# HaoxiangYou/Q_Learning_with_HJB

Measured on AMD Instinct MI355X. Metric: env-steps/sec (batched HJB rollouts), cartpole batch=2^20, higher is better.
Workload: dtype f32; 1 GPU; cartpole balancing + vhjb controller (BASELINE configs[1]); batch_per_gpu=1048576, global_batch=1048576, state_dim=4, control_dim=1, integrator=euler, mlp=4-128-128-64 relu, no bias, parallelism=env-shard x1, no data-path collective

## Files before the change

### q_learning_with_hjb_amd/csrc/hjbx_mlp_host.hpp

```cpp
#pragma once
#include <type_traits>

#include "hjbx_host.hpp"
#include "hjbx_mlp_kernels.hpp"
#include "hjbx_hessian_kernels.hpp"

inline hjbx_net make_net(const hjbx_mlp* mlp) {
    return hjbx_net{0, mlp->activation, mlp->h1, mlp->h2, mlp->h3, mlp->mean, mlp->std, mlp->xf, mlp->eps_scalar, (const float*)mlp->W1,
                    (const float*)mlp->W2, (const float*)mlp->W3, nullptr, nullptr, nullptr, nullptr, nullptr};
}
inline hjbx_net make_net(const hjbx_softpd_mlp* mlp) {
    return hjbx_net{1, mlp->activation, mlp->h1, mlp->h2, mlp->h3, mlp->mean, mlp->std, mlp->xf, 0.0, (const float*)mlp->W1, (const float*)mlp->W2,
                    (const float*)mlp->W3, (const float*)mlp->b1, (const float*)mlp->b2, (const float*)mlp->b3, (const float*)mlp->w4, (const float*)mlp->b4};
}

template <int N> inline MlpP<N> make_mlp_params(const hjbx_net& net) {
    MlpP<N> p;
    for (int k = 0; k < N; ++k) { p.mean[k] = (float)net.mean[k]; p.istd[k] = (float)(1.0 / net.std[k]); p.xf[k] = (float)net.xf[k]; }
    p.eps_s = (float)net.eps_scalar;
    return p;
}

template <typename Head> inline Head make_head(const hjbx_net& net) {
    if constexpr (std::is_same<Head, MlpHeadSoft>::value) return MlpHeadSoft{net.b1, net.b2, net.b3, net.w4, net.b4};
    else return MlpHeadPd{};
}

static constexpr int kEmptyCall = 1;

inline int check_features(const char* who, const hjbx_net& net) {
    if (net.h1 != kH1 || net.h2 != kH2 || net.h3 != kH3)
        return hjbx_set_error(HJBX_EUNSUPPORTED, "%s: features must be [128,128,64], got [%d,%d,%d]", who, net.h1, net.h2, net.h3);
    if (net.activation != HJBX_ACT_RELU && net.activation != HJBX_ACT_TANH && net.activation != HJBX_ACT_SIN)
        return hjbx_set_error(HJBX_EINVAL, "%s: unknown activation %d", who, net.activation);
    return HJBX_OK;
}
inline int check_std(const char* who, const hjbx_net& net, int n) {
    for (int k = 0; k < n; ++k)
        if (!(net.std[k] != 0.0)) return hjbx_set_error(HJBX_EINVAL, "%s: normalization_std[%d] is zero", who, k);
    return HJBX_OK;
}
inline bool state_rows_aligned(const void* p, const hjbx_system* sys) { return aligned_rows(p, (size_t)sys->n * sizeof(float), 7u); }
inline int check_net(const char* who, const hjbx_system* sys, const hjbx_net& net) {
    if (net.soft) {
        if (!net.W1 || !net.b1 || !net.W2 || !net.b2 || !net.W3 || !net.b3 || !net.w4 || !net.b4)
            return hjbx_set_error(HJBX_EINVAL, "%s: NULL weight or bias pointer", who);
        if (sys->kind == HJBX_SYS_USER && !hjbx_user_matrix_cores(sys))
            return hjbx_set_error(HJBX_EUNSUPPORTED, "%s: the matrix-core kernels exist for the built-in systems only", who);
    }
    return check_features(who, net);
}

inline int check_value_grad(const char* who, const hjbx_system* sys, const hjbx_net& net, const float* x, const float* V, const float* g, int64_t B) {
    if (B < 0) return hjbx_set_error(HJBX_EINVAL, "%s: negative batch size", who);
    if (B == 0 || (!V && !g)) return kEmptyCall;
    if (net.soft ? !x : (!x || !net.W1 || !net.W2 || !net.W3))
        return hjbx_set_error(HJBX_EINVAL, net.soft ? "%s: NULL x" : "%s: NULL x or weight pointer", who);
    if (int rc = check_net(who, sys, net)) return rc;
    if (!state_rows_aligned(x, sys) || (g && !state_rows_aligned(g, sys)))
        return hjbx_set_error(HJBX_EINVAL, "%s: x / gradV must be aligned to their row vector width", who);
    return check_std(who, net, sys->n);
}

inline int check_value_hessian(const char* who, const hjbx_system* sys, const hjbx_net& net, const float* x, const float* H, const float* dy, int64_t B) {
    if (B < 0) return hjbx_set_error(HJBX_EINVAL, "%s: negative batch size", who);
    if (B == 0 || (!H && !dy)) return kEmptyCall;
    if (!x || !net.W1 || !net.W2 || !net.W3 || (net.soft && (!net.b1 || !net.b2 || !net.b3 || !net.w4 || !net.b4)))
        return hjbx_set_error(HJBX_EINVAL, net.soft ? "%s: NULL x, weight or bias pointer" : "%s: NULL x or weight pointer", who);
    if (sys->kind == HJBX_SYS_USER && !hjbx_user_matrix_cores(sys))
        return hjbx_set_error(HJBX_EUNSUPPORTED, "%s: user-defined systems are not supported unless the handle has asked for the matrix-core kernels "
                                                 "(hjbx_system_enable_matrix_cores)", who);
    if (int rc = check_features(who, net)) return rc;
    if (!state_rows_aligned(x, sys) || (reinterpret_cast<uintptr_t>(H) & 15u) || (reinterpret_cast<uintptr_t>(dy) & 15u))
        return hjbx_set_error(HJBX_EINVAL, net.soft ? "%s: x must be aligned to its row vector width, H to 16 bytes"
                                                    : "%s: x must be aligned to its row vector width, H and dy_dx to 16 bytes", who);
    return check_std(who, net, sys->n);
}

inline int check_rollout(const char* who, const hjbx_system* sys, const hjbx_task* task, const hjbx_net& net, const hjbx_rollout_args& a) {
    if (int rc = check_task(task)) return rc;
    if (a.B < 0 || a.n_steps < 0 || a.t_first < 0 || a.T_max < 0) return hjbx_set_error(HJBX_EINVAL, "%s: negative size or step index", who);
    if (int rc = check_integrator(sys, a.integrator, who)) return rc;
    if (a.B == 0) return kEmptyCall;
    if (!a.x || !a.cost || !a.done || !a.done_step || (!net.soft && (!net.W1 || !net.W2 || !net.W3)))
        return hjbx_set_error(HJBX_EINVAL, net.soft ? "%s: x, cost, done and done_step must be non-NULL" : "%s: x, cost, done, done_step and the weights must be non-NULL", who);
    if (!a.workspace || (reinterpret_cast<uintptr_t>(a.workspace) & 15u))
        return hjbx_set_error(HJBX_EINVAL, "%s: workspace must be a 16-byte aligned device buffer of hjbx_rollout_workspace_bytes() zero-filled bytes", who);
    if (int rc = check_net(who, sys, net)) return rc;
    if (!state_rows_aligned(a.x, sys) || (a.traj && !state_rows_aligned(a.traj, sys)) || (a.x_out && !state_rows_aligned(a.x_out, sys)) ||
        (a.u_log && !aligned_rows(a.u_log, (size_t)sys->m * sizeof(float))))
        return hjbx_set_error(HJBX_EINVAL, "%s: x / traj / x_out / u_log must be aligned to their row vector width", who);
    return check_std(who, net, sys->n);
}

inline int mlp_persistent_grid(int64_t B, int per_group, int64_t* ngroups, int64_t* grid, const char* who) {
    *ngroups = (B + per_group - 1) / per_group;
    const int n_cu = hjbx_device_cus();
    if (n_cu <= 0) return hjbx_set_error(HJBX_ENODEVICE, "%s: no HIP device", who);
    *grid = *ngroups < n_cu ? *ngroups : n_cu;
    return HJBX_OK;
}

inline int mlp_rollout_grid(int64_t B, int64_t* ngroups, int64_t* grid, int* sched, const char* who) {
    if (int rc = mlp_persistent_grid(B, 32, ngroups, grid, who)) return rc;
    *sched = hjbx_option_value(HJBX_OPT_ROLLOUT_SCHEDULE);
    *grid += hjbx_option_value(HJBX_OPT_ROLLOUT_EXTRA_WORKGROUPS);
    if (*grid > kMaxGrid) *grid = kMaxGrid;
    return HJBX_OK;
}

template <typename S, int TL, int WAVES, int ACT, int ARITH, typename Head>
int launch_value_grad(S sys, const hjbx_net& net, const float* x, float* V, float* g, int64_t B, void* st, const char* who) {
    const MlpP<S::N> p = make_mlp_params<S::N>(net);
    int64_t ngroups = 0, grid = 0;
    if (int rc = mlp_persistent_grid(B, 32 * TL, &ngroups, &grid, who)) return rc;
    hipLaunchKernelGGL((k_value_grad_mfma<S, TL, WAVES, ACT, ARITH, Head>), dim3((unsigned)grid), dim3(WAVES * 64), 0, (hipStream_t)st, sys, p, net.W1,
                       net.W2, net.W3, x, V, g, B, ngroups, make_head<Head>(net));
    hipError_t e = hipGetLastError();
    if (e != hipSuccess) return hjbx_set_error(HJBX_EHIP, "%s: %s", who, hipGetErrorString(e));
    return HJBX_OK;
}

template <typename S, int ACT, typename Head>
int launch_value_hessian(S sys, const hjbx_net& net, const float* x, float* H, float* dy, int64_t B, void* st, const char* who) {
    const MlpP<S::N> p = make_mlp_params<S::N>(net);
    int64_t ngroups = 0, grid = 0;
    if (int rc = mlp_persistent_grid(B, 32 / S::N, &ngroups, &grid, who)) return rc;
    hipLaunchKernelGGL((k_value_hessian<S, kHessWaves, ACT, Head>), dim3((unsigned)grid), dim3(kHessWaves * 64), 0, (hipStream_t)st, sys, p, net.W1,
                       net.W2, net.W3, x, H, dy, B, ngroups, make_head<Head>(net));
    hipError_t e = hipGetLastError();
    if (e != hipSuccess) return hjbx_set_error(HJBX_EHIP, "%s: %s", who, hipGetErrorString(e));
    return HJBX_OK;
}

template <typename S, int WAVES, int ACT, int ARITH, typename Head>
int launch_rollout(const hjbx_system* sysh, S sys, const hjbx_task* task, const hjbx_net& net, const hjbx_rollout_args& a, const char* who) {
    constexpr int N = S::N, M = S::M;
    const MlpP<N> p = make_mlp_params<N>(net);
    const auto tk = make_task<float, N, M>(task);
    const auto lim = make_limits<float, M>(sysh);
    RolloutOut<N, M> o{a.traj, a.u_log, a.cost, a.done, a.resid, a.done_step, a.x_out};
    int64_t ngroups = 0, grid = 0;
    int sched = 0;
    if (int rc = mlp_rollout_grid(a.B, &ngroups, &grid, &sched, who)) return rc;
    auto launch = [&](auto integ) {
        hipLaunchKernelGGL((k_vhjb_rollout_mfma<decltype(integ)::value, S, WAVES, ACT, ARITH, Head>), dim3((unsigned)grid), dim3(WAVES * 64), 0,
                           (hipStream_t)a.stream, sys, p, tk, lim, net.W1, net.W2, net.W3, a.t_first, a.n_steps, a.T_max, a.x, a.env_order, o, a.B, ngroups,
                           (unsigned*)a.workspace, sched, make_head<Head>(net));
    };
    if (a.integrator == HJBX_EULER) launch(std::integral_constant<int, 0>{});
    else if (a.integrator == HJBX_RK4) launch(std::integral_constant<int, 1>{});
    else if constexpr (S::kHasZoh) launch(std::integral_constant<int, 2>{});
    hipError_t e = hipGetLastError();
    if (e != hipSuccess) return hjbx_set_error(HJBX_EHIP, "%s: %s", who, hipGetErrorString(e));
    return HJBX_OK;
}

template <typename Go> int dispatch_value_system(const hjbx_system* sys, const char* who, Go go) {
    switch (sys->kind) {
    case HJBX_SYS_CARTPOLE: return go(Cartpole<float>{});
#if !defined(HJBX_MLP_DEV) || defined(HJBX_MLP_DEV_QUAD2D)
    case HJBX_SYS_QUAD2D: return go(Quad2D<float>{});
#endif
#ifndef HJBX_MLP_DEV
    case HJBX_SYS_LINEAR:
        if (sys->n == 2) return go(Linear<float, 2, 1>{});
        if (sys->n == 4) return go(Linear<float, 4, 1>{});
        if (sys->n == 6) return go(Linear<float, 6, 2>{});
        break;
    case HJBX_SYS_ACROBOT: return go(Acrobot<float>{});
    case HJBX_SYS_NEARHOVER: return go(NearHover<float>{});
#endif
    }
    return hjbx_set_error(HJBX_EUNSUPPORTED, "%s: no kernel for system kind %d with n=%d", who, sys->kind, sys->n);
}
template <int TL, int WAVES, int ACT, int ARITH, typename Head>
int dispatch_value_grad(const hjbx_system* sys, const hjbx_net& net, const float* x, float* V, float* g, int64_t B, void* st, const char* who) {
    return dispatch_value_system(sys, who, [&](auto s) { return launch_value_grad<decltype(s), TL, WAVES, ACT, ARITH, Head>(s, net, x, V, g, B, st, who); });
}
template <int ACT, typename Head>
int dispatch_value_hessian(const hjbx_system* sys, const hjbx_net& net, const float* x, float* H, float* dy, int64_t B, void* st, const char* who) {
    return dispatch_value_system(sys, who, [&](auto s) { return launch_value_hessian<decltype(s), ACT, Head>(s, net, x, H, dy, B, st, who); });
}

template <int WAVES, int ACT, int ARITH, typename Head>
int dispatch_rollout(const hjbx_system* sys, const hjbx_task* task, const hjbx_net& net, const hjbx_rollout_args& a, const char* who) {
    int rc = HJBX_EUNSUPPORTED;
    const bool ok = with_system<float>(sys, [&](auto S) {
        using SS = decltype(S);
#ifdef HJBX_MLP_DEV
        if constexpr (std::is_same<SS, Cartpole<float>>::value)
#else
        if constexpr (SS::N % 2 == 0)
#endif
            rc = launch_rollout<SS, WAVES, ACT, ARITH, Head>(sys, S, task, net, a, who);
    });
    if (!ok || rc == HJBX_EUNSUPPORTED) return hjbx_set_error(HJBX_EUNSUPPORTED, "%s: no kernel for system kind %d with n=%d m=%d", who, sys->kind, sys->n, sys->m);
    return rc;
}

using mlp_value_grad_fn = int(const hjbx_system* sys, const hjbx_net& net, const float* x, float* V, float* g, int64_t B, void* stream, const char* who);
using mlp_rollout_fn = int(const hjbx_system* sys, const hjbx_task* task, const hjbx_net& net, const hjbx_rollout_args& a, const char* who);
using mlp_value_hessian_fn = int(const hjbx_system* sys, const hjbx_net& net, const float* x, float* H, float* dy, int64_t B, void* stream, const char* who);
#define HJBX_MLP_SYM2(prefix, name, v) prefix##name##v
#define HJBX_MLP_SYM(prefix, name, v) HJBX_MLP_SYM2(prefix, name, v)
#define HJBX_MLP_DECLARE_VARIANT(prefix, v)                                                          \
    __attribute__((visibility("hidden"))) mlp_value_grad_fn HJBX_MLP_SYM(prefix, _value_grad_act, v); \
    __attribute__((visibility("hidden"))) mlp_rollout_fn HJBX_MLP_SYM(prefix, _rollout_act, v);
#define HJBX_MLP_DEFINE_VARIANT(prefix, v, TL, WAVES, ACT, ARITH, Head)                                                                            \
    int HJBX_MLP_SYM(prefix, _value_grad_act, v)(const hjbx_system* sys, const hjbx_net& net, const float* x, float* V, float* g, int64_t B,        \
                                                 void* stream, const char* who) {                                                                  \
        return dispatch_value_grad<TL, WAVES, ACT, ARITH, Head>(sys, net, x, V, g, B, stream, who);                                                \
    }                                                                                                                                              \
    int HJBX_MLP_SYM(prefix, _rollout_act, v)(const hjbx_system* sys, const hjbx_task* task, const hjbx_net& net, const hjbx_rollout_args& a,       \
                                              const char* who) {                                                                                   \
        return dispatch_rollout<WAVES, ACT, ARITH, Head>(sys, task, net, a, who);                                                                  \
    }
#define HJBX_HESS_DECLARE_VARIANT(prefix, v) __attribute__((visibility("hidden"))) mlp_value_hessian_fn HJBX_MLP_SYM(prefix, _value_hessian_act, v);
#define HJBX_HESS_DEFINE_VARIANT(prefix, v, ACT, Head)                                                                                              \
    int HJBX_MLP_SYM(prefix, _value_hessian_act, v)(const hjbx_system* sys, const hjbx_net& net, const float* x, float* H, float* dy, int64_t B,    \
                                                    void* stream, const char* who) {                                                               \
        return dispatch_value_hessian<ACT, Head>(sys, net, x, H, dy, B, stream, who);                                                              \
    }
```

### q_learning_with_hjb_amd/csrc/hjbx_mlp_kernels.hpp

```cpp
#pragma once
#include <hip/hip_runtime.h>
#include <type_traits>

#include <cstddef>

#include "hjbx_internal.hpp"
#include "hjbx_systems.hpp"
#include "hjbx_mlp_core.hpp"
#include "hjbx_mlp_x3.hpp"
#include "hjbx_mlp_h2.hpp"

using namespace hjbx;

struct MlpHeadPd {
    static constexpr bool kSoft = false;
    template <int N, int AR> using Lds = typename MlpArith<AR>::template Lds<N>;
};
struct MlpHeadSoft {
    static constexpr bool kSoft = true;
    template <int N, int AR> using Lds = MlpLdsSoft<N>;
    const float *b1, *b2, *b3, *w4, *b4;
};

template <typename S, int TL, int WAVES, int ACT, int AR, typename HEAD = MlpHeadPd>
__global__ __launch_bounds__(WAVES * 64, WAVES / 4) void k_value_grad_mfma(S sys, MlpP<S::N> p, const float* __restrict__ W1g,
                                                                         const float* __restrict__ W2g, const float* __restrict__ W3g,
                                                                         const float* __restrict__ x, float* __restrict__ Vout,
                                                                         float* __restrict__ gout, int64_t B, int64_t ngroups, HEAD head) {
    constexpr int N = S::N;
    static_assert(N % 2 == 0, "state dimension must be even (k-steps of 2)");
    static_assert(AR == 0 || TL == 1, "the split-operand chains hold one tile per wave");
    __shared__ __attribute__((aligned(256))) typename HEAD::template Lds<N, AR> L;
    const int tid = threadIdx.x;
    if (tid == 0) L.next = WAVES;
#ifdef HJBX_DIAG_CLOCK
    const unsigned long long tentry = __builtin_amdgcn_s_memrealtime();
#endif
    MlpArith<AR>::template fill<N, WAVES * 64>(L, W1g, W2g, W3g, tid);
    if constexpr (HEAD::kSoft) mlp_fill_bias<WAVES * 64>(L.bias, head.b1, head.b2, head.b3, head.w4, head.b4, tid);
    __syncthreads();
    const int lane = tid & 63, wave = tid >> 6;
    const auto c = [&] { return MlpArith<AR>::template ctx<N>(L, lane); }();
    const int i = c.i, h = c.h;

    const int64_t groups_per_wg = (ngroups + gridDim.x - 1) / gridDim.x;
    const int64_t g_begin = (int64_t)blockIdx.x * groups_per_wg;
    const int64_t g_end = (g_begin + groups_per_wg < ngroups) ? g_begin + groups_per_wg : ngroups;

    auto load_rows = [&](int64_t grp, float (&dst)[TL][N]) {
#pragma unroll
        for (int t = 0; t < TL; ++t) {
            const int64_t en = (grp * TL + t) * 32 + i;
            load_sample<N>(x, p, en, grp < g_end && en < B, dst[t]);
        }
    };

    int64_t grp = g_begin + wave;
#ifdef HJBX_DIAG_CLOCK
    const unsigned long long t0c = __builtin_amdgcn_s_memtime(), t0r = __builtin_amdgcn_s_memrealtime();
#endif
    float xs[TL][N], xn[TL][N];
    load_rows(grp, xs);
    for (; grp < g_end;) {
        asm volatile("" ::: "memory");
        int nxt = 0;
        if (lane == 0) nxt = atomicAdd(&L.next, 1);
        const int64_t grp_next = g_begin + __builtin_amdgcn_readfirstlane(nxt);
        load_rows(grp_next, xn);

        float V[TL], g[TL][N];
        if constexpr (HEAD::kSoft) mlp_value_grad<S, TL, ACT, true>(sys, p, c, xs, gout != nullptr, V, g, &L.bias);
        else MlpArith<AR>::template value_grad<S, TL, ACT>(sys, p, c, xs, gout != nullptr, V, g);
#pragma unroll
        for (int t = 0; t < TL; ++t) {
            const int64_t env = (grp * TL + t) * 32 + i;
            if (env < B && h == 0) {
#ifndef HJBX_DIAG_CLOCK
                if (Vout) Vout[env] = V[t];
#endif
                if (gout) store_row<N>(gout, env, g[t]);
            }
#pragma unroll
            for (int k = 0; k < N; ++k) xs[t][k] = xn[t][k];
        }
        grp = grp_next;
    }
#ifdef HJBX_DIAG_CLOCK
    {
        const unsigned long long t1c = __builtin_amdgcn_s_memtime(), t1r = __builtin_amdgcn_s_memrealtime();
        if (Vout && gout && lane == 0) {
            float* d = Vout + 4 * ((int64_t)blockIdx.x * WAVES + wave);
            d[0] = (float)(t1c - t0c); d[1] = (float)(t1r - t0r);
            d[2] = (float)(t0r - tentry); d[3] = (float)(tentry & 0xFFFFFFull);
        }
    }
#endif
}

template <int N, int M> struct RolloutOut {
    float* traj;
    float* u_log;
    float* cost;
    float* done;
    float* resid;
    int32_t* done_step;
    float* x_out;
};

static constexpr int kWsQueue = 0;
static constexpr int kWsStarted = 32;
static constexpr int kWsExited = 64;
static constexpr int kWsFlags = 96;
static constexpr int kMaxGrid = 1024;
static constexpr int kWsOpen = kWsFlags + kMaxGrid;
static constexpr int kWsWords = kWsOpen + kMaxGrid;
#define HJBX_RLX_AGENT __ATOMIC_RELAXED, __HIP_MEMORY_SCOPE_AGENT

template <int INTEG, typename S, int WAVES, int ACT, int AR, typename HEAD = MlpHeadPd>
__global__ __launch_bounds__(WAVES * 64, WAVES / 4) void k_vhjb_rollout_mfma(S sys_k, MlpP<S::N> p_k, TaskP<float, S::N, S::M> tk_k,
                                                                           Limits<float, S::M> lim_k, const float* __restrict__ W1g,
                                                                           const float* __restrict__ W2g, const float* __restrict__ W3g,
                                                                           int t_first, int n_steps, int T_max, const float* x ,
                                                                           const int32_t* __restrict__ order, RolloutOut<S::N, S::M> o, int64_t B,
                                                                           int64_t ngroups, unsigned* ws, int sched, HEAD head) {
    constexpr int N = S::N, M = S::M;
    static_assert(N % 2 == 0, "state dimension must be even (k-steps of 2)");
    __shared__ __attribute__((aligned(256))) typename HEAD::template Lds<N, AR> L;
    __shared__ __attribute__((aligned(16))) unsigned char sys_raw[sizeof(S)];
    S& sys_s = *reinterpret_cast<S*>(sys_raw);
    __shared__ MlpP<N> p_s;
    __shared__ TaskP<float, N, M> tk_s;
    __shared__ Limits<float, M> lim_s;
    const int tid = threadIdx.x;
    __shared__ int q_next[4];
    __shared__ int waves_done;
    __shared__ unsigned my_flag;
    if (tid < 4) q_next[tid] = WAVES / 4;
    if (tid == 0) {
        waves_done = 0;
        unsigned seen = 0u;
        __hip_atomic_compare_exchange_strong(ws + kWsFlags + blockIdx.x, &seen, 1u, __ATOMIC_RELAXED, HJBX_RLX_AGENT);
        my_flag = seen;
        __hip_atomic_fetch_add(ws + kWsStarted, 1u, HJBX_RLX_AGENT);
        sys_s = sys_k; p_s = p_k; tk_s = tk_k; lim_s = lim_k;
    }
    MlpArith<AR>::template fill<N, WAVES * 64>(L, W1g, W2g, W3g, tid);
    if constexpr (HEAD::kSoft) mlp_fill_bias<WAVES * 64>(L.bias, head.b1, head.b2, head.b3, head.w4, head.b4, tid);
    __syncthreads();
    const S& sys = sys_s;
    const MlpP<N>& p = p_s;
    const TaskP<float, N, M>& tk = tk_s;
    const Limits<float, M>& lim = lim_s;
    const int lane = tid & 63, wave = __builtin_amdgcn_readfirstlane(tid >> 6);
    const unsigned my_flag_u = (unsigned)__builtin_amdgcn_readfirstlane((int)my_flag);
    const auto c = [&] { return MlpArith<AR>::template ctx<N>(L, lane); }();
    const int i = c.i, h = c.h;
    const int simd = wave & 3;
    const int G = (int)gridDim.x;
    const int64_t picks_per_wg = (ngroups + G - 1) / G;
    auto group_of = [&](int w, int64_t pick) -> int64_t {
        if (pick >= picks_per_wg) return -1;
        const int64_t g = order ? (int64_t)w + pick * G : (int64_t)w * picks_per_wg + pick;
        return g < ngroups ? g : -1;
    };
    int victim = -1;
    auto next_group = [&]() -> int64_t {
        if (sched == 1) {
            unsigned t = 0;
            if (lane == 0) t = __hip_atomic_fetch_add(ws + kWsQueue, 1u, HJBX_RLX_AGENT);
            const int64_t g = (int64_t)G * WAVES + (unsigned)__builtin_amdgcn_readfirstlane((int)t);
            return g < ngroups ? g : -1;
        }
        if (victim < 0) {
            int nxt = 0;
            if (lane == 0) nxt = atomicAdd(&q_next[simd], 1);
            const int64_t g = my_flag_u == 0u ? group_of(blockIdx.x, simd + 4 * (int64_t)__builtin_amdgcn_readfirstlane(nxt)) : -1;
            if (g >= 0) return g;
            victim = 0;
            unsigned started = 0;
            if (lane == 0) started = __hip_atomic_load(ws + kWsStarted, HJBX_RLX_AGENT);
            if (__builtin_amdgcn_readfirstlane((int)started) >= G) victim = G;
        }
        while (victim < G) {
            const int w = victim + lane;
            unsigned f = 1u;
            if (w < G) {
                f = __hip_atomic_load(ws + kWsFlags + w, HJBX_RLX_AGENT);
                if (f == 0u && __hip_atomic_compare_exchange_strong(ws + kWsFlags + w, &f, 2u, __ATOMIC_RELAXED, HJBX_RLX_AGENT)) f = 2u;
            }
            unsigned long long open = __builtin_amdgcn_ballot_w64(f == 2u);
            while (open) {
                const int b = __builtin_ctzll(open);
                unsigned t = 0;
                if (lane == 0) t = __hip_atomic_fetch_add(ws + kWsOpen + victim + b, 1u, HJBX_RLX_AGENT);
                const int64_t g = group_of(victim + b, (int64_t)(unsigned)__builtin_amdgcn_readfirstlane((int)t));
                if (g >= 0) { victim += b; return g; }
                open &= open - 1;
            }
            victim = (victim + 64 < G) ? victim + 64 : G;
        }
        return -1;
    };
    int64_t grp;
    if (sched == 1) grp = (int64_t)blockIdx.x * WAVES + wave < ngroups ? (int64_t)blockIdx.x * WAVES + wave : -1;
    else grp = my_flag_u == 0u ? group_of(blockIdx.x, wave) : -1;
    if (grp < 0) grp = next_group();
    while (grp >= 0) {
        const int64_t slot = grp * 32 + i;
        const bool valid = slot < B;
        int64_t env = valid ? (order ? (int64_t)order[slot] : slot) : 0;
        env = env < 0 ? 0 : (env >= B ? B - 1 : env);
        const bool writer = valid && h == 0;
        float xs[1][N];
        int32_t ds = 0;
        if (valid) {
            load_row<N>(x, env, xs[0]);
            ds = o.done_step[env];
        } else {
#pragma unroll
            for (int k = 0; k < N; ++k) xs[0][k] = p.xf[k];
        }
        if (o.traj && writer) store_row<N>(o.traj, env, xs[0]);
        for (int k = 0; k < n_steps; ++k) {
            asm volatile("" ::: "memory");
            float xo[N], u[M], cst, dn, res;
            if (__builtin_amdgcn_ballot_w64(ds < 0) == 0) {
#pragma unroll
                for (int q = 0; q < N; ++q) xo[q] = xs[0][q];
#pragma unroll
                for (int j = 0; j < M; ++j) u[j] = 0.0f;
                cst = dn = res = 0.0f;
            } else {
                float V[1], g[1][N];
                if constexpr (HEAD::kSoft) mlp_value_grad<S, 1, ACT, true>(sys, p, c, xs, true, V, g, &L.bias);
                else MlpArith<AR>::template value_grad<S, 1, ACT>(sys, p, c, xs, true, V, g);
                vhjb_step_env<INTEG>(sys, tk, lim, t_first + k, T_max, o.resid != nullptr, xs[0], g[0], ds, xo, u, cst, dn, res);
            }
            if (writer) {
                const int64_t row = (int64_t)k * B + env;
                o.cost[row] = cst;
                o.done[row] = dn;
                if (o.resid) o.resid[row] = res;
                if (o.u_log) store_row<M>(o.u_log + (int64_t)k * B * M, env, u);
                if (o.traj) store_row<N>(o.traj + (int64_t)(k + 1) * B * N, env, xo);
            }
#pragma unroll
            for (int q = 0; q < N; ++q) xs[0][q] = xo[q];
        }
        if (writer) {
            o.done_step[env] = ds;
            if (o.x_out) store_row<N>(o.x_out, env, xs[0]);
        }
        grp = next_group();
    }
    int lastw = 0;
    if (lane == 0 && atomicAdd(&waves_done, 1) == WAVES - 1) lastw = __hip_atomic_fetch_add(ws + kWsExited, 1u, HJBX_RLX_AGENT) == (unsigned)(G - 1);
    if (__builtin_amdgcn_readfirstlane(lastw)) {
        for (int w = lane; w < kWsWords; w += 64)
            if (w < kWsFlags || (w - kWsFlags) % kMaxGrid < G) __hip_atomic_store(ws + w, 0u, HJBX_RLX_AGENT);
    }
}
```

### q_learning_with_hjb_amd/csrc/hjbx_user.hip

```cpp
#include <hip/hip_runtime.h>
#include <hip/hiprtc.h>

#include <dlfcn.h>
#include <elf.h>

#include <cstdio>
#include <cstring>
#include <map>
#include <mutex>
#include <new>
#include <string>
#include <vector>

#include "hjbx_internal.hpp"
#include "hjbx_host.hpp"
#include "hjbx_mlp_kernels.hpp"
#include "hjbx_mlp_host.hpp"

#define HJBX_EMBEDDED_HEADERS(X)                                                    \
    X(hjbx_src_systems, "hjbx_systems.hpp", "hjbx_systems.hpp")                     \
    X(hjbx_src_stream, "hjbx_stream_kernels.hpp", "hjbx_stream_kernels.hpp")        \
    X(hjbx_src_user, "hjbx_user_kernels.hpp", "hjbx_user_kernels.hpp")              \
    X(hjbx_src_user_mlp, "hjbx_user_mlp_kernels.hpp", "hjbx_user_mlp_kernels.hpp")  \
    X(hjbx_src_mlp_core, "hjbx_mlp_core.hpp", "hjbx_mlp_core.hpp")                  \
    X(hjbx_src_mlp_kernels, "hjbx_mlp_kernels.hpp", "hjbx_mlp_kernels.hpp")         \
    X(hjbx_src_mlp_x3, "hjbx_mlp_x3.hpp", "hjbx_mlp_x3.hpp")                        \
    X(hjbx_src_mlp_h2, "hjbx_mlp_h2.hpp", "hjbx_mlp_h2.hpp")                        \
    X(hjbx_src_train_coop, "hjbx_train_coop_kernels.hpp", "hjbx_train_coop_kernels.hpp") \
    X(hjbx_src_user_train, "hjbx_user_train_kernels.hpp", "hjbx_user_train_kernels.hpp") \
    X(hjbx_src_hessian_kernels, "hjbx_hessian_kernels.hpp", "hjbx_hessian_kernels.hpp") \
    X(hjbx_src_user_hessian, "hjbx_user_hessian_kernels.hpp", "hjbx_user_hessian_kernels.hpp") \
    X(hjbx_src_abi, "../../include/hjbx.h", "hjbx.h")
#if !defined(__HIP_DEVICE_COMPILE__)
#ifndef HJBX_CSRC_DIR
#error "compile hjbx_user.hip with -DHJBX_CSRC_DIR=\"<absolute path of csrc>\""
#endif
#define HJBX_EMBED(sym, file, name)                                                                                               \
    asm(".pushsection .rodata\n.global " #sym "\n.type " #sym ", @object\n" #sym ":\n.incbin \"" HJBX_CSRC_DIR "/" file "\"\n.byte 0\n" \
        ".popsection\n");
HJBX_EMBEDDED_HEADERS(HJBX_EMBED)
#undef HJBX_EMBED
#endif
#define HJBX_DECLARE(sym, file, name) extern "C" const char sym[];
HJBX_EMBEDDED_HEADERS(HJBX_DECLARE)
#undef HJBX_DECLARE

static const char kStubRuntime[] = "// hip/hip_runtime.h: provided by hiprtc itself\n";
static const char kStubStdint[] =
    "#pragma once\n"
    "typedef signed char int8_t; typedef unsigned char uint8_t; typedef short int16_t; typedef unsigned short uint16_t;\n"
    "typedef int int32_t; typedef unsigned int uint32_t; typedef long int64_t; typedef unsigned long uint64_t; typedef unsigned long uintptr_t;\n";
static const char kStubStddef[] =
    "#pragma once\n"
    "typedef unsigned long size_t;\n"
    "#ifndef offsetof\n#define offsetof(t, m) __builtin_offsetof(t, m)\n#endif\n";
static const char kStubTypeTraits[] =
    "#pragma once\n"
    "namespace std {\n"
    "template <bool C, class A, class B> struct conditional { using type = A; };\n"
    "template <class A, class B> struct conditional<false, A, B> { using type = B; };\n"
    "template <bool C, class A, class B> using conditional_t = typename conditional<C, A, B>::type;\n"
    "template <class T, T v> struct integral_constant { static constexpr T value = v; };\n"
    "}\n";
static const char kStubInternal[] = "#pragma once\n#include \"hjbx.h\"\n";

namespace {
struct Rtc {
    decltype(&hiprtcCreateProgram) create = nullptr;
    decltype(&hiprtcCompileProgram) compile = nullptr;
    decltype(&hiprtcGetProgramLogSize) log_size = nullptr;
    decltype(&hiprtcGetProgramLog) log = nullptr;
    decltype(&hiprtcGetCodeSize) code_size = nullptr;
    decltype(&hiprtcGetCode) code = nullptr;
    decltype(&hiprtcDestroyProgram) destroy = nullptr;
    decltype(&hiprtcAddNameExpression) add_name = nullptr;
    decltype(&hiprtcGetLoweredName) lowered = nullptr;
    bool ok = false;
};

const Rtc& rtc() {
    static Rtc r;
    static std::once_flag once;
    std::call_once(once, [] {
        void* h = nullptr;
        for (const char* name : {"libhiprtc.so.7", "libhiprtc.so", "/opt/rocm/lib/libhiprtc.so"}) {
            h = dlopen(name, RTLD_NOW | RTLD_GLOBAL);
            if (h) break;
        }
        if (!h) return;
#define HJBX_SYM(field, sym) r.field = reinterpret_cast<decltype(r.field)>(dlsym(h, #sym))
        HJBX_SYM(create, hiprtcCreateProgram); HJBX_SYM(compile, hiprtcCompileProgram); HJBX_SYM(log_size, hiprtcGetProgramLogSize);
        HJBX_SYM(log, hiprtcGetProgramLog); HJBX_SYM(code_size, hiprtcGetCodeSize); HJBX_SYM(code, hiprtcGetCode);
        HJBX_SYM(destroy, hiprtcDestroyProgram); HJBX_SYM(add_name, hiprtcAddNameExpression); HJBX_SYM(lowered, hiprtcGetLoweredName);
#undef HJBX_SYM
        r.ok = r.create && r.compile && r.log_size && r.log && r.code_size && r.code && r.destroy && r.add_name && r.lowered;
    });
    return r;
}

thread_local std::string g_compile_log;

struct UserUnit {
    std::vector<char> code;
    hipModule_t mod[kMaxDevices] = {};
    std::map<std::string, hipFunction_t> fn[kMaxDevices];
    int state = 0, status = HJBX_OK;
    std::string error, log;
    std::string kernel[4];
};

struct UserProgram {
    std::mutex mu;
    UserUnit stream;
    std::string source;
    int user_kind = 0, n = 0, m = 0, np = 1;
    std::mutex mc_mu;
    bool matrix_cores = false;
    UserUnit mc[2][3];
    std::mutex train_mu;
    UserUnit train[3];
    std::mutex hess_mu;
    UserUnit hess[2][3];
};

int compile_unit(const Rtc& R, const char* who, const char* top, const char* unit_name, const std::string& snippet, int user_kind, int n, int m,
                 int np, const std::vector<std::string>& extra, const std::vector<const char*>& name_exprs, UserUnit* out) {
#define HJBX_TEXT(sym, file, name) sym,
#define HJBX_NAME(sym, file, name) name,
    const char* headers[] = {HJBX_EMBEDDED_HEADERS(HJBX_TEXT) kStubInternal, snippet.c_str(), kStubRuntime, kStubStdint, kStubStddef, kStubStddef,
                             kStubTypeTraits};
    const char* names[] = {HJBX_EMBEDDED_HEADERS(HJBX_NAME) "hjbx_internal.hpp", "hjbx_user_snippet.hpp", "hip/hip_runtime.h", "stdint.h", "stddef.h",
                           "cstddef", "type_traits"};
#undef HJBX_TEXT
#undef HJBX_NAME
    static_assert(sizeof(headers) == sizeof(names), "one name per header");
    hiprtcProgram prog = nullptr;
    if (R.create(&prog, top, unit_name, (int)(sizeof(headers) / sizeof(headers[0])), headers, names) != HIPRTC_SUCCESS)
        return hjbx_set_error(HJBX_EHIP, "%s: hiprtcCreateProgram failed", who);
    for (const char* e : name_exprs)
        if (R.add_name(prog, e) != HIPRTC_SUCCESS) { R.destroy(&prog); return hjbx_set_error(HJBX_EHIP, "%s: hiprtcAddNameExpression(%s) failed", who, e); }
    std::vector<std::string> o = {"--offload-arch=gfx950", "-O3", "-std=c++17", "-ffp-contract=on", "-DHJBX_USER_N=" + std::to_string(n),
                                  "-DHJBX_USER_M=" + std::to_string(m), "-DHJBX_USER_NP=" + std::to_string(np),
                                  "-DHJBX_USER_KIND=" + std::to_string(user_kind)};
    o.insert(o.end(), extra.begin(), extra.end());
    std::vector<const char*> opts;
    for (const std::string& f : o) opts.push_back(f.c_str());
    const hiprtcResult rc = R.compile(prog, (int)opts.size(), opts.data());
    size_t ls = 0;
    if (R.log_size(prog, &ls) == HIPRTC_SUCCESS && ls > 1) {
        g_compile_log.resize(ls);
        if (R.log(prog, &g_compile_log[0]) != HIPRTC_SUCCESS) g_compile_log.clear();
    }
    if (rc != HIPRTC_SUCCESS) {
        R.destroy(&prog);
        return hjbx_set_error(HJBX_EINVAL, "%s: the device source does not compile (hjbx_last_compile_log has the compiler's messages): %.300s", who,
                              g_compile_log.c_str());
    }
    size_t cs = 0;
    if (R.code_size(prog, &cs) != HIPRTC_SUCCESS || cs == 0) { R.destroy(&prog); return hjbx_set_error(HJBX_EHIP, "%s: no code object", who); }
    out->code.resize(cs);
    hiprtcResult rg = R.code(prog, out->code.data());
    for (size_t i = 0; rg == HIPRTC_SUCCESS && i < name_exprs.size() && i < 4; ++i) {
        const char* low = nullptr;
        rg = R.lowered(prog, name_exprs[i], &low);
        if (rg == HIPRTC_SUCCESS && low) out->kernel[i] = low;
    }
    R.destroy(&prog);
    if (rg != HIPRTC_SUCCESS) { out->code.clear(); return hjbx_set_error(HJBX_EHIP, "%s: hiprtcGetCode / hiprtcGetLoweredName failed", who); }
    return HJBX_OK;
}

long kernel_scratch_bytes(const std::vector<char>& code, const std::string& kernel) {
    Elf64_Ehdr eh;
    if (code.size() < sizeof eh) return -1;
    memcpy(&eh, code.data(), sizeof eh);
    if (memcmp(eh.e_ident, ELFMAG, SELFMAG) != 0 || eh.e_ident[EI_CLASS] != ELFCLASS64 || eh.e_shentsize != sizeof(Elf64_Shdr)) return -1;
    if (eh.e_shoff > code.size() || (size_t)eh.e_shnum * sizeof(Elf64_Shdr) > code.size() - eh.e_shoff) return -1;
    std::vector<Elf64_Shdr> sh(eh.e_shnum);
    if (eh.e_shnum) memcpy(sh.data(), code.data() + eh.e_shoff, sh.size() * sizeof(Elf64_Shdr));
    auto inside = [&](const Elf64_Shdr& s) { return s.sh_offset <= code.size() && s.sh_size <= code.size() - s.sh_offset; };
    const std::string want = kernel + ".kd";
    for (const Elf64_Shdr& st : sh) {
        if ((st.sh_type != SHT_SYMTAB && st.sh_type != SHT_DYNSYM) || st.sh_link >= sh.size() || !inside(st) || !inside(sh[st.sh_link])) continue;
        const Elf64_Shdr& str = sh[st.sh_link];
        for (size_t k = 0; k + sizeof(Elf64_Sym) <= st.sh_size; k += sizeof(Elf64_Sym)) {
            Elf64_Sym sym;
            memcpy(&sym, code.data() + st.sh_offset + k, sizeof sym);
            if (sym.st_name >= str.sh_size || sym.st_shndx >= sh.size()) continue;
            const char* nm = code.data() + str.sh_offset + sym.st_name;
            if (strnlen(nm, str.sh_size - sym.st_name) != want.size() || memcmp(nm, want.data(), want.size()) != 0) continue;
            const Elf64_Shdr& sec = sh[sym.st_shndx];
            if (!inside(sec) || sym.st_value < sec.sh_addr || sym.st_value - sec.sh_addr + 8 > sec.sh_size) return -1;
            uint32_t priv = 0;
            memcpy(&priv, code.data() + sec.sh_offset + (sym.st_value - sec.sh_addr) + 4, 4);
            return (long)priv;
        }
    }
    return -1;
}

int launch_unit(UserProgram* u, UserUnit& unit, const char* kernel, unsigned grid, unsigned block, void** args, void* stream, const char* who) {
    const int dev = hjbx_current_device();
    if (dev < 0) return hjbx_set_error(HJBX_ENODEVICE, "%s: no HIP device", who);
    hipFunction_t f = nullptr;
    {
        std::lock_guard<std::mutex> lock(u->mu);
        if (!unit.mod[dev]) {
            const hipError_t e = hipModuleLoadData(&unit.mod[dev], unit.code.data());
            if (e != hipSuccess) { unit.mod[dev] = nullptr; return hjbx_set_error(HJBX_EHIP, "hipModuleLoadData: %s", hipGetErrorString(e)); }
        }
        auto it = unit.fn[dev].find(kernel);
        if (it == unit.fn[dev].end()) {
            const hipError_t e = hipModuleGetFunction(&f, unit.mod[dev], kernel);
            if (e != hipSuccess) return hjbx_set_error(HJBX_EHIP, "hipModuleGetFunction(%s): %s", kernel, hipGetErrorString(e));
            unit.fn[dev][kernel] = f;
        } else {
            f = it->second;
        }
    }
    const hipError_t e = hipModuleLaunchKernel(f, grid, 1, 1, block, 1, 1, 0, (hipStream_t)stream, args, nullptr);
    if (e != hipSuccess) return hjbx_set_error(HJBX_EHIP, "%s: %s", who, hipGetErrorString(e));
    return HJBX_OK;
}

void unload_unit(UserUnit& unit) {
    for (int d = 0; d < kMaxDevices; ++d)
        if (unit.mod[d]) (void)hipModuleUnload(unit.mod[d]);
}

struct UnitSpec {
    const char *top, *name;
    std::vector<std::string> flags;
    std::vector<const char*> kernels, labels;
    std::string variant;
    const char* budget;
};

template <typename MakeSpec> int lazy_unit(UserProgram* u, UserUnit& unit, MakeSpec&& make_spec, const char* who, UserUnit** out) {
    if (unit.state == 0) {
        const UnitSpec spec = make_spec();
        g_compile_log.clear();
        const Rtc& R = rtc();
        int rc = compile_unit(R, who, spec.top, spec.name, u->source, u->user_kind, u->n, u->m, u->np, spec.flags, spec.kernels, &unit);
        for (size_t k = 0; rc == HJBX_OK && k < spec.kernels.size(); ++k) {
            const long scratch = kernel_scratch_bytes(unit.code, unit.kernel[k]);
            if (scratch < 0) rc = hjbx_set_error(HJBX_EHIP, "%s: kernel %s is missing from the compiled code object", who, unit.kernel[k].c_str());
            else if (scratch > 0)
                rc = hjbx_set_error(HJBX_EUNSUPPORTED, "%s: the %s kernel of this user system (n=%d m=%d, %s) needs %ld bytes of scratch: its code does not fit %s",
                                    who, spec.labels[k], u->n, u->m, spec.variant.c_str(), scratch, spec.budget);
        }
        unit.state = rc == HJBX_OK ? 1 : -1;
        unit.status = rc;
        unit.log = g_compile_log;
        if (rc != HJBX_OK) {
            char msg[512];
            hjbx_last_error(msg, sizeof msg);
            unit.error = msg;
            unit.code.clear();
        }
    }
    if (unit.state < 0) {
        g_compile_log = unit.log;
        return hjbx_set_error(unit.status, "%s", unit.error.c_str());
    }
    *out = &unit;
    return HJBX_OK;
}

int matrix_core_unit(const hjbx_system* s, int soft, int act, const char* who, UserUnit** out) {
    UserProgram* u = s->kind == HJBX_SYS_USER ? static_cast<UserProgram*>(s->user) : nullptr;
    if (!u) return hjbx_set_error(HJBX_EINVAL, "%s: not a user-defined system", who);
    if (soft < 0 || soft > 1 || act < 0 || act > 2) return hjbx_set_error(HJBX_EINVAL, "%s: unknown head %d / activation %d", who, soft, act);
    std::lock_guard<std::mutex> lock(u->mc_mu);
    if (!u->matrix_cores)
        return hjbx_set_error(HJBX_EUNSUPPORTED, "%s: this user-defined system has not asked for the matrix-core kernels (hjbx_system_enable_matrix_cores)", who);
    return lazy_unit(u, u->mc[soft][act], [&] { return
                     UnitSpec{"#include \"hjbx_user_mlp_kernels.hpp\"\n", "hjbx_user_matrix_cores.hip",
                              {"-DHJBX_USER_MLP_ACT=" + std::to_string(act), "-DHJBX_USER_MLP_SOFT=" + std::to_string(soft)},
                              {"HJBX_UM_VALUE_GRAD", "HJBX_UM_ROLLOUT_EULER", "HJBX_UM_ROLLOUT_RK4"}, {"value-gradient", "Euler rollout", "RK4 rollout"},
                              "activation " + std::to_string(act) + (soft ? ", soft-PD head" : ", PD head"), "the 256 registers of the matrix-core kernels"}; },
                     who, out);
}

int train_unit(const hjbx_system* s, int act, const char* who, UserUnit** out) {
    UserProgram* u = s->kind == HJBX_SYS_USER ? static_cast<UserProgram*>(s->user) : nullptr;
    if (!u) return hjbx_set_error(HJBX_EINVAL, "%s: not a user-defined system", who);
    if (act < 0 || act > 2) return hjbx_set_error(HJBX_EINVAL, "%s: unknown activation %d", who, act);
    if (s->n % 2)
        return hjbx_set_error(HJBX_EUNSUPPORTED, "%s: the fused parameter gradient needs an even state dimension (k-steps of 2), got n=%d", who, s->n);
    if (!hjbx_user_matrix_cores(s))
        return hjbx_set_error(HJBX_EUNSUPPORTED, "%s: this user-defined system has not asked for the matrix-core kernels (hjbx_system_enable_matrix_cores)", who);
    if (act == HJBX_ACT_SIN && s->n > 4)
        return hjbx_set_error(HJBX_EUNSUPPORTED, "%s: the sin network's fused parameter gradient exists for n <= 4 (n = %d)", who, s->n);
    std::lock_guard<std::mutex> lock(u->train_mu);
    return lazy_unit(u, u->train[act], [&] { return
                     UnitSpec{"#include \"hjbx_user_train_kernels.hpp\"\n", "hjbx_user_train.hip", {"-DHJBX_USER_MLP_ACT=" + std::to_string(act)},
                              {"HJBX_UT_M0_PS1", "HJBX_UT_M0_PS4", "HJBX_UT_M1_PS1", "HJBX_UT_M1_PS4"},
                              {"k_train_coop<mode 0, PS 1>", "k_train_coop<mode 0, PS 4>", "k_train_coop<mode 1, PS 1>", "k_train_coop<mode 1, PS 4>"},
                              "activation " + std::to_string(act),
                              "the 512 registers of the cooperative parameter-gradient kernel; the fused parameter gradient is refused for this system"}; },
                     who, out);
}

int hessian_unit(const hjbx_system* s, int soft, int act, const char* who, UserUnit** out) {
    UserProgram* u = s->kind == HJBX_SYS_USER ? static_cast<UserProgram*>(s->user) : nullptr;
    if (!u) return hjbx_set_error(HJBX_EINVAL, "%s: not a user-defined system", who);
    if (soft < 0 || soft > 1 || act < 0 || act > 2) return hjbx_set_error(HJBX_EINVAL, "%s: unknown head %d / activation %d", who, soft, act);
    if (!hjbx_user_matrix_cores(s))
        return hjbx_set_error(HJBX_EUNSUPPORTED, "%s: this user-defined system has not asked for the matrix-core kernels (hjbx_system_enable_matrix_cores)", who);
    if (soft && act == HJBX_ACT_RELU)
        return hjbx_set_error(HJBX_EUNSUPPORTED, "%s: the Hessian of a soft-PD ReLU network is identically zero (H is filled with zeros): there is no kernel and no code object", who);
    std::lock_guard<std::mutex> lock(u->hess_mu);
    return lazy_unit(u, u->hess[soft][act], [&] { return
                     UnitSpec{"#include \"hjbx_user_hessian_kernels.hpp\"\n", "hjbx_user_hessian.hip",
                              {"-DHJBX_USER_MLP_ACT=" + std::to_string(act), "-DHJBX_USER_MLP_SOFT=" + std::to_string(soft)},
                              {"HJBX_UH_VALUE_HESSIAN"}, {"value-Hessian"},
                              "activation " + std::to_string(act) + (soft ? ", soft-PD head" : ", PD head"), "the 512 registers of the Hessian kernel"}; },
                     who, out);
}
}

extern "C" size_t hjbx_last_compile_log(char* buf, size_t buflen) {
    const size_t len = g_compile_log.size();
    if (buf && buflen) {
        const size_t n = len < buflen - 1 ? len : buflen - 1;
        memcpy(buf, g_compile_log.data(), n);
        buf[n] = '\0';
    }
    return len;
}

void hjbx_user_release(void* up) {
    UserProgram* u = static_cast<UserProgram*>(up);
    if (!u) return;
    unload_unit(u->stream);
    for (auto& head : u->mc)
        for (UserUnit& unit : head) unload_unit(unit);
    for (UserUnit& unit : u->train) unload_unit(unit);
    for (auto& head : u->hess)
        for (UserUnit& unit : head) unload_unit(unit);
    delete u;
}

extern "C" int hjbx_system_create_from_source(int user_kind, const char* device_source, int n, int m, double dt, const double* umin,
                                              const double* umax, const double* params, int n_params, hjbx_system** out) {
    if (!out) return hjbx_set_error(HJBX_EINVAL, "out is NULL");
    *out = nullptr;
    g_compile_log.clear();
    if (user_kind != HJBX_USER_AFFINE && user_kind != HJBX_USER_MANIPULATOR) return hjbx_set_error(HJBX_EINVAL, "unknown user system kind %d", user_kind);
    if (!device_source || !umin || !umax) return hjbx_set_error(HJBX_EINVAL, "device_source / umin / umax must be non-NULL");
    if (n < 1 || n > HJBX_MAX_N || m < 1 || m > HJBX_MAX_M) return hjbx_set_error(HJBX_EINVAL, "user system needs 1<=n<=%d, 1<=m<=%d", HJBX_MAX_N, HJBX_MAX_M);
    if (user_kind == HJBX_USER_MANIPULATOR && n % 2) return hjbx_set_error(HJBX_EINVAL, "a manipulator state is (q, dq): n must be even, got %d", n);
    if (n_params < 0 || n_params > HJBX_USER_MAX_PARAMS || (n_params > 0 && !params))
        return hjbx_set_error(HJBX_EINVAL, "user system takes 0..%d parameters", HJBX_USER_MAX_PARAMS);
    if (!(dt > 0) || !(dt < 1e300)) return hjbx_set_error(HJBX_EINVAL, "dt must be positive and finite");
    for (int j = 0; j < m; ++j)
        if (!(umin[j] <= umax[j])) return hjbx_set_error(HJBX_EINVAL, "umin[%d] > umax[%d]", j, j);
    const Rtc& R = rtc();
    if (!R.ok) {
        const char* why = dlerror();
        return hjbx_set_error(HJBX_EUNSUPPORTED, "hjbx_system_create_from_source: libhiprtc.so could not be loaded (%s)", why ? why : "symbols missing");
    }
    UserProgram* u = new (std::nothrow) UserProgram();
    if (!u) return hjbx_set_error(HJBX_EINVAL, "out of host memory");
    u->source = device_source; u->user_kind = user_kind; u->n = n; u->m = m; u->np = n_params > 0 ? n_params : 1;
    if (int rc = compile_unit(R, "hjbx_system_create_from_source", "#include \"hjbx_user_kernels.hpp\"\n", "hjbx_user_system.hip", u->source, user_kind,
                              n, m, u->np, {}, {}, &u->stream)) {
        delete u;
        return rc;
    }
    hjbx_system* s = new_system(HJBX_SYS_USER, n, m, dt, umin, umax, params, n_params, u);
    if (!s) { delete u; return hjbx_set_error(HJBX_EINVAL, "out of host memory"); }
    *out = s;
    return HJBX_OK;
}

extern "C" int hjbx_system_enable_matrix_cores(hjbx_system* sys) {
    if (!sys) return hjbx_set_error(HJBX_EINVAL, "hjbx_system_enable_matrix_cores: system handle is NULL");
    UserProgram* u = sys->kind == HJBX_SYS_USER ? static_cast<UserProgram*>(sys->user) : nullptr;
    if (!u) return hjbx_set_error(HJBX_EINVAL, "hjbx_system_enable_matrix_cores: a built-in system has its matrix-core kernels already (user-defined systems only)");
    if (sys->n % 2)
        return hjbx_set_error(HJBX_EUNSUPPORTED, "hjbx_system_enable_matrix_cores: the matrix-core kernels need an even state dimension (k-steps of 2), got n=%d", sys->n);
    if (sys->n > HJBX_MAX_N || sys->m > HJBX_MAX_M)
        return hjbx_set_error(HJBX_EUNSUPPORTED, "hjbx_system_enable_matrix_cores: the matrix-core kernels take n<=%d, m<=%d", HJBX_MAX_N, HJBX_MAX_M);
    std::lock_guard<std::mutex> lock(u->mc_mu);
    u->matrix_cores = true;
    return HJBX_OK;
}

bool hjbx_user_matrix_cores(const hjbx_system* s) {
    UserProgram* u = s && s->kind == HJBX_SYS_USER ? static_cast<UserProgram*>(s->user) : nullptr;
    if (!u) return false;
    std::lock_guard<std::mutex> lock(u->mc_mu);
    return u->matrix_cores;
}

extern "C" int hjbx_system_matrix_cores(const hjbx_system* sys) { return hjbx_user_matrix_cores(sys) ? 1 : 0; }

extern "C" size_t hjbx_system_code_object(const hjbx_system* sys, int which, void* buf, size_t len) {
    UserProgram* u = sys && sys->kind == HJBX_SYS_USER ? static_cast<UserProgram*>(sys->user) : nullptr;
    if (!u) { hjbx_set_error(HJBX_EINVAL, "hjbx_system_code_object: not a user-defined system"); return 0; }
    const UserUnit* unit = &u->stream;
    if (which != HJBX_CODE_STREAMING) {
        if (which < 1 || which > 15) { hjbx_set_error(HJBX_EINVAL, "hjbx_system_code_object: unknown code object %d", which); return 0; }
        UserUnit* mc = nullptr;
        if (which >= 10) {
            if (hessian_unit(sys, (which - 10) / 3, (which - 10) % 3, "hjbx_system_code_object", &mc) != HJBX_OK) return 0;
        } else if (which >= 7) {
            if (train_unit(sys, which - 7, "hjbx_system_code_object", &mc) != HJBX_OK) return 0;
        } else if (matrix_core_unit(sys, (which - 1) / 3, (which - 1) % 3, "hjbx_system_code_object", &mc) != HJBX_OK) {
            return 0;
        }
        unit = mc;
    }
    if (buf && len) memcpy(buf, unit->code.data(), len < unit->code.size() ? len : unit->code.size());
    return unit->code.size();
}

int hjbx_user_launch(const hjbx_system* s, const char* kernel, unsigned grid, void** args, void* stream) {
    UserProgram* u = static_cast<UserProgram*>(s->user);
    if (!u) return hjbx_set_error(HJBX_EINVAL, "system handle has no user program");
    return launch_unit(u, u->stream, kernel, grid, 256, args, stream, kernel);
}

namespace {
constexpr unsigned kMcBlock = 8 * 64;
}

int hjbx_user_value_grad(const hjbx_system* s, const hjbx_net& net, const float* x, float* V, float* g, int64_t B, void* stream, const char* who) {
    UserUnit* unit = nullptr;
    if (int rc = matrix_core_unit(s, net.soft, net.activation, who, &unit)) return rc;
    return with_mc_dims(s, who, "matrix-core kernel", [&](auto Nc, auto) -> int {
        constexpr int N = decltype(Nc)::value;
        auto blob = user_blob<float>(s);
        MlpP<N> p = make_mlp_params<N>(net);
        int64_t ngroups = 0, grid = 0;
        if (int rc = mlp_persistent_grid(B, 32, &ngroups, &grid, who)) return rc;
        MlpHeadSoft soft = make_head<MlpHeadSoft>(net);
        MlpHeadPd pd{};
        void* a[] = {&blob, &p, (void*)&net.W1, (void*)&net.W2, (void*)&net.W3, (void*)&x, (void*)&V, (void*)&g, (void*)&B, &ngroups,
                     net.soft ? (void*)&soft : (void*)&pd};
        return launch_unit(static_cast<UserProgram*>(s->user), *unit, unit->kernel[0].c_str(), (unsigned)grid, kMcBlock, a, stream, who);
    });
}

int hjbx_user_rollout(const hjbx_system* s, const hjbx_task* task, const hjbx_net& net, const hjbx_rollout_args& r, const char* who) {
    if (r.integrator != HJBX_EULER && r.integrator != HJBX_RK4) return hjbx_set_error(HJBX_EUNSUPPORTED, "%s: a user system steps with HJBX_EULER or HJBX_RK4", who);
    UserUnit* unit = nullptr;
    if (int rc = matrix_core_unit(s, net.soft, net.activation, who, &unit)) return rc;
    return with_mc_dims(s, who, "matrix-core kernel", [&](auto Nc, auto Mc) -> int {
        constexpr int N = decltype(Nc)::value, M = decltype(Mc)::value;
        auto blob = user_blob<float>(s);
        MlpP<N> p = make_mlp_params<N>(net);
        auto tk = make_task<float, N, M>(task);
        auto lim = make_limits<float, M>(s);
        RolloutOut<N, M> o{r.traj, r.u_log, r.cost, r.done, r.resid, r.done_step, r.x_out};
        int64_t ngroups = 0, grid = 0;
        int sched = 0;
        if (int rc = mlp_rollout_grid(r.B, &ngroups, &grid, &sched, who)) return rc;
        unsigned* ws = (unsigned*)r.workspace;
        MlpHeadSoft soft = make_head<MlpHeadSoft>(net);
        MlpHeadPd pd{};
        void* a[] = {&blob, &p, &tk, &lim, (void*)&net.W1, (void*)&net.W2, (void*)&net.W3, (void*)&r.t_first, (void*)&r.n_steps, (void*)&r.T_max, (void*)&r.x,
                     (void*)&r.env_order, &o, (void*)&r.B, &ngroups, &ws, &sched, net.soft ? (void*)&soft : (void*)&pd};
        return launch_unit(static_cast<UserProgram*>(s->user), *unit, unit->kernel[r.integrator == HJBX_RK4 ? 2 : 1].c_str(), (unsigned)grid, kMcBlock, a,
                           r.stream, who);
    });
}

int hjbx_user_value_hessian(const hjbx_system* s, const hjbx_net& net, const float* x, float* H, float* dy, int64_t B, void* stream, const char* who) {
    UserUnit* unit = nullptr;
    if (int rc = hessian_unit(s, net.soft, net.activation, who, &unit)) return rc;
    return with_mc_dims(s, who, "Hessian kernel", [&](auto Nc, auto) -> int {
        constexpr int N = decltype(Nc)::value;
        auto blob = user_blob<float>(s);
        MlpP<N> p = make_mlp_params<N>(net);
        int64_t ngroups = 0, grid = 0;
        if (int rc = mlp_persistent_grid(B, 32 / N, &ngroups, &grid, who)) return rc;
        MlpHeadSoft soft = make_head<MlpHeadSoft>(net);
        MlpHeadPd pd{};
        void* a[] = {&blob, &p, (void*)&net.W1, (void*)&net.W2, (void*)&net.W3, (void*)&x, (void*)&H, (void*)&dy, (void*)&B, &ngroups,
                     net.soft ? (void*)&soft : (void*)&pd};
        return launch_unit(static_cast<UserProgram*>(s->user), *unit, unit->kernel[0].c_str(), (unsigned)grid, kHessWaves * 64, a, stream, who);
    });
}

int hjbx_user_train_unit(const hjbx_system* s, int activation, const char* who) {
    UserUnit* unit = nullptr;
    return train_unit(s, activation, who, &unit);
}

int hjbx_user_train_launch(const hjbx_system* s, int activation, int mode, int psplit, unsigned grid, void** args, void* stream, const char* who) {
    if (mode < 0 || mode > 1 || (psplit != 1 && psplit != 4)) return hjbx_set_error(HJBX_EINVAL, "%s: residual mode %d / psplit %d", who, mode, psplit);
    UserUnit* unit = nullptr;
    if (int rc = train_unit(s, activation, who, &unit)) return rc;
    return launch_unit(static_cast<UserProgram*>(s->user), *unit, unit->kernel[2 * mode + (psplit == 4 ? 1 : 0)].c_str(), grid, 256, args, stream, who);
}
```

Baseline: 1.410 billion env-steps/s.

## Give each wave lane its own env in rollout, evaluating MLP in two tiles

Before this change, each group of 32 envs was handled by a 64-lane wave with duplicated halves, and only the h==0 half wrote results. Now every lane owns a distinct env, so a group holds 64 envs. The MLP value/gradient is evaluated over two 32-env tiles, with states gathered via ds_bpermute and a tile skipped when all its envs are done. Each lane then steps its own env. This removes the redundant half-wave dynamics and writes, and halves the number of groups, at the cost of a serialised two-pass MLP loop and extra permute traffic; user matrix-core units keep the old 32-env layout.

```diff
diff --git a/q_learning_with_hjb_amd/csrc/hjbx_mlp_host.hpp b/q_learning_with_hjb_amd/csrc/hjbx_mlp_host.hpp
--- a/q_learning_with_hjb_amd/csrc/hjbx_mlp_host.hpp
+++ b/q_learning_with_hjb_amd/csrc/hjbx_mlp_host.hpp
@@ -101,8 +101,8 @@
     return HJBX_OK;
 }
 
-inline int mlp_rollout_grid(int64_t B, int64_t* ngroups, int64_t* grid, int* sched, const char* who) {
-    if (int rc = mlp_persistent_grid(B, 32, ngroups, grid, who)) return rc;
+inline int mlp_rollout_grid(int64_t B, int group_envs, int64_t* ngroups, int64_t* grid, int* sched, const char* who) {
+    if (int rc = mlp_persistent_grid(B, group_envs, ngroups, grid, who)) return rc;
     *sched = hjbx_option_value(HJBX_OPT_ROLLOUT_SCHEDULE);
     *grid += hjbx_option_value(HJBX_OPT_ROLLOUT_EXTRA_WORKGROUPS);
     if (*grid > kMaxGrid) *grid = kMaxGrid;
@@ -142,7 +142,7 @@
     RolloutOut<N, M> o{a.traj, a.u_log, a.cost, a.done, a.resid, a.done_step, a.x_out};
     int64_t ngroups = 0, grid = 0;
     int sched = 0;
-    if (int rc = mlp_rollout_grid(a.B, &ngroups, &grid, &sched, who)) return rc;
+    if (int rc = mlp_rollout_grid(a.B, kRolloutGroupEnvs, &ngroups, &grid, &sched, who)) return rc;
     auto launch = [&](auto integ) {
         hipLaunchKernelGGL((k_vhjb_rollout_mfma<decltype(integ)::value, S, WAVES, ACT, ARITH, Head>), dim3((unsigned)grid), dim3(WAVES * 64), 0,
                            (hipStream_t)a.stream, sys, p, tk, lim, net.W1, net.W2, net.W3, a.t_first, a.n_steps, a.T_max, a.x, a.env_order, o, a.B, ngroups,
diff --git a/q_learning_with_hjb_amd/csrc/hjbx_mlp_kernels.hpp b/q_learning_with_hjb_amd/csrc/hjbx_mlp_kernels.hpp
--- a/q_learning_with_hjb_amd/csrc/hjbx_mlp_kernels.hpp
+++ b/q_learning_with_hjb_amd/csrc/hjbx_mlp_kernels.hpp
@@ -115,6 +115,13 @@
 static constexpr int kWsOpen = kWsFlags + kMaxGrid;
 static constexpr int kWsWords = kWsOpen + kMaxGrid;
 #define HJBX_RLX_AGENT __ATOMIC_RELAXED, __HIP_MEMORY_SCOPE_AGENT
+
+#ifdef HJBX_USER_MATRIX_CORE_UNIT
+static constexpr bool kRolloutPairs = false;
+#else
+static constexpr bool kRolloutPairs = true;
+#endif
+static constexpr int kRolloutGroupEnvs = kRolloutPairs ? 64 : 32;
 
 template <int INTEG, typename S, int WAVES, int ACT, int AR, typename HEAD = MlpHeadPd>
 __global__ __launch_bounds__(WAVES * 64, WAVES / 4) void k_vhjb_rollout_mfma(S sys_k, MlpP<S::N> p_k, TaskP<float, S::N, S::M> tk_k,
@@ -206,11 +213,11 @@
     else grp = my_flag_u == 0u ? group_of(blockIdx.x, wave) : -1;
     if (grp < 0) grp = next_group();
     while (grp >= 0) {
-        const int64_t slot = grp * 32 + i;
+        const int64_t slot = grp * kRolloutGroupEnvs + (kRolloutPairs ? lane : i);
         const bool valid = slot < B;
         int64_t env = valid ? (order ? (int64_t)order[slot] : slot) : 0;
         env = env < 0 ? 0 : (env >= B ? B - 1 : env);
-        const bool writer = valid && h == 0;
+        const bool writer = kRolloutPairs ? valid : valid && h == 0;
         float xs[1][N];
         int32_t ds = 0;
         if (valid) {
@@ -224,12 +231,30 @@
         for (int k = 0; k < n_steps; ++k) {
             asm volatile("" ::: "memory");
             float xo[N], u[M], cst, dn, res;
-            if (__builtin_amdgcn_ballot_w64(ds < 0) == 0) {
+            const unsigned long long live = __builtin_amdgcn_ballot_w64(ds < 0);
+            if (live == 0) {
 #pragma unroll
                 for (int q = 0; q < N; ++q) xo[q] = xs[0][q];
 #pragma unroll
                 for (int j = 0; j < M; ++j) u[j] = 0.0f;
                 cst = dn = res = 0.0f;
+            } else if constexpr (kRolloutPairs) {
+                float gs[N];
+#pragma unroll
+                for (int q = 0; q < N; ++q) gs[q] = 0.0f;
+#pragma clang loop unroll(disable)
+                for (int tile = 0; tile < 2; ++tile) {
+                    if ((unsigned)(live >> (32 * tile)) == 0u) continue;
+                    const int src = (i | (tile << 5)) << 2;
+                    float xt[1][N], V[1], g[1][N];
+#pragma unroll
+                    for (int q = 0; q < N; ++q) xt[0][q] = __builtin_bit_cast(float, __builtin_amdgcn_ds_bpermute(src, __builtin_bit_cast(int, xs[0][q])));
+                    if constexpr (HEAD::kSoft) mlp_value_grad<S, 1, ACT, true>(sys, p, c, xt, true, V, g, &L.bias);
+                    else MlpArith<AR>::template value_grad<S, 1, ACT>(sys, p, c, xt, true, V, g);
+#pragma unroll
+                    for (int q = 0; q < N; ++q) gs[q] = h == tile ? g[0][q] : gs[q];
+                }
+                vhjb_step_env<INTEG>(sys, tk, lim, t_first + k, T_max, o.resid != nullptr, xs[0], gs, ds, xo, u, cst, dn, res);
             } else {
                 float V[1], g[1][N];
                 if constexpr (HEAD::kSoft) mlp_value_grad<S, 1, ACT, true>(sys, p, c, xs, true, V, g, &L.bias);
diff --git a/q_learning_with_hjb_amd/csrc/hjbx_user.hip b/q_learning_with_hjb_amd/csrc/hjbx_user.hip
--- a/q_learning_with_hjb_amd/csrc/hjbx_user.hip
+++ b/q_learning_with_hjb_amd/csrc/hjbx_user.hip
@@ -457,7 +457,7 @@
         RolloutOut<N, M> o{r.traj, r.u_log, r.cost, r.done, r.resid, r.done_step, r.x_out};
         int64_t ngroups = 0, grid = 0;
         int sched = 0;
-        if (int rc = mlp_rollout_grid(r.B, &ngroups, &grid, &sched, who)) return rc;
+        if (int rc = mlp_rollout_grid(r.B, 32, &ngroups, &grid, &sched, who)) return rc;
         unsigned* ws = (unsigned*)r.workspace;
         MlpHeadSoft soft = make_head<MlpHeadSoft>(net);
         MlpHeadPd pd{};
```

Result: slower. 735.6 million env-steps/s (-47.8%).
